# nadeemlab/DeepLIIF

Hardware: AMD Instinct MI355X
Metric: 512x512 tiles/s train-step (5G+5D) (higher is better)
Workload: dtype bf16; 1 GPU; DeepLIIF train step, 5x Resnet-9block G + 5x NLayerD(n=4), GAN+SmoothL1+Adam (BASELINE configs[2] per GPU); tile=512x512x3, batch_per_gpu=8, global_batch=8, norm=instance, precision_policy=bf16, parallelism=dp1, rccl_ranks=1, backend=nccl, streams=3

## Files before the change

deepliif_amd/csrc/conv_s2f.hip:

```cpp
#include "conv_args.h"

__device__ __attribute__((aligned(64))) unsigned char g_s2f_zero_page[64];

constexpr int S2F_MAX_OFF = 9;
struct S2fArgs {
    ConvArgs a;
    int n_off;
    int off_delta[S2F_MAX_OFF];
    int8_t off_dh[S2F_MAX_OFF], off_dw[S2F_MAX_OFF];
    int user_k[S2F_MAX_OFF][4];
};

__device__ __forceinline__ float s2f_row16_sum(float v) {
    v += __builtin_bit_cast(float, __builtin_amdgcn_update_dpp(0, __builtin_bit_cast(int, v), 0xB1, 0xf, 0xf, false));
    v += __builtin_bit_cast(float, __builtin_amdgcn_update_dpp(0, __builtin_bit_cast(int, v), 0x4E, 0xf, 0xf, false));
    v += __builtin_bit_cast(float, __builtin_amdgcn_update_dpp(0, __builtin_bit_cast(int, v), 0x141, 0xf, 0xf, false));
    v += __builtin_bit_cast(float, __builtin_amdgcn_update_dpp(0, __builtin_bit_cast(int, v), 0x140, 0xf, 0xf, false));
    return v;
}

constexpr int S2F_XB = 256 * 128;
constexpr int S2F_WB = 64 * 128;
constexpr int S2F_BUF = S2F_XB + 4 * S2F_WB;
constexpr size_t S2F_LOOP_LDS = (size_t)2 * S2F_BUF;
constexpr size_t S2F_EPI_LDS = (size_t)256 * 512 + 256 * sizeof(int) + (size_t)4 * 2 * 64 * sizeof(float);
constexpr size_t S2F_LDS = S2F_LOOP_LDS > S2F_EPI_LDS ? S2F_LOOP_LDS : S2F_EPI_LDS;

__global__ void __launch_bounds__(512) conv_s2f_kernel(const S2fArgs sa) {
    const ConvArgs &a = sa.a;
    extern __shared__ __attribute__((aligned(16))) char smem_raw[];
    lds_char_t *lds = (lds_char_t *)smem_raw;

    const int tid = threadIdx.x, lane = tid & 63;
    const int wave = __builtin_amdgcn_readfirstlane(tid >> 6);
    const int wm = wave & 3, wn = wave >> 2;
    const int bid = xcd_remap(blockIdx.x, gridDim.x);
    const int tn = bid % a.tiles_n, tm = bid / a.tiles_n;
    const int nch = a.Ci >> 6;
    const int NO = sa.n_off;
    const int T = nch * NO;

    const int lrow = lane >> 3, lcp = lane & 7;
    const int HWq = a.Hq * a.Wq;
    const bf16_t *in = reinterpret_cast<const bf16_t *>(a.in);
    const bf16_t *zero = reinterpret_cast<const bf16_t *>(g_s2f_zero_page);
    const bf16_t *x_ptr[4];
    unsigned x_mask[4];
#pragma unroll
    for (int i = 0; i < 4; ++i) {
        const int s = (wave * 4 + i) * 8 + lrow;
        const int m = tm * 256 + s;
        const bool ok = m < a.Mtot;
        const int mm = ok ? m : 0;
        const int n = mm / HWq, rem = mm - n * HWq;
        const int hq = rem / a.Wq, wq = rem - hq * a.Wq;
        x_ptr[i] = in + ((size_t)(n * a.Hi + hq) * a.Wi + wq) * (size_t)a.in_pstride + (lcp ^ ((s >> 1) & 7)) * 8;
        unsigned mk = 0;
        if (ok)
            for (int o = 0; o < NO; ++o) {
                const int hi = hq + sa.off_dh[o], wi = wq + sa.off_dw[o];
                if (((unsigned)hi < (unsigned)a.Hi) && ((unsigned)wi < (unsigned)a.Wi)) mk |= 1u << o;
            }
        x_mask[i] = mk;
    }
    const int wrow = wave * 8 + lrow;
    const bf16_t *w_ptr = a.w_hi + (size_t)(tn * 64 + wrow) * a.w_kstride + (lcp ^ ((wrow >> 1) & 7)) * 8;

    auto stage = [&](int u) __attribute__((always_inline)) {
        const int c = u / NO, o = u - c * NO;
        const int buf = (u & 1) * S2F_BUF;
        const ptrdiff_t xd = (ptrdiff_t)sa.off_delta[o] + c * 64;
#pragma unroll
        for (int i = 0; i < 4; ++i) {
            const bool ok = (x_mask[i] >> o) & 1u;
            const bf16_t *src = ok ? x_ptr[i] + xd : zero;
            __builtin_amdgcn_global_load_lds((const __attribute__((address_space(1))) void *)src,
                                             (__attribute__((address_space(3))) void *)(lds + buf + (wave * 4 + i) * 1024), 16, 0, 0);
        }
#pragma unroll
        for (int p = 0; p < 4; ++p) {
            const int kb = sa.user_k[o][p];
            if (kb >= 0)
                __builtin_amdgcn_global_load_lds((const __attribute__((address_space(1))) void *)(w_ptr + kb + c * 64),
                                                 (__attribute__((address_space(3))) void *)(lds + buf + S2F_XB + p * S2F_WB + wave * 1024), 16, 0, 0);
        }
    };

    const int lr = lane & 31, lh = lane >> 5;
    const int ax = (wm * 64 + lr) * 128 + ((lh ^ ((lr >> 1) & 7)) << 4);
    const int aw = S2F_XB + (wn * 32 + lr) * 128 + ((lh ^ ((lr >> 1) & 7)) << 4);

    f32x16_t acc[4][2];
#pragma unroll
    for (int p = 0; p < 4; ++p)
#pragma unroll
        for (int j = 0; j < 2; ++j)
#pragma unroll
            for (int r = 0; r < 16; ++r) acc[p][j][r] = 0.f;

    if (T > 0) stage(0);
    for (int u = 0; u < T; ++u) {
        asm volatile("s_waitcnt vmcnt(0)\n\ts_barrier" ::: "memory");
        if (u + 1 < T) stage(u + 1);
        const int c = u / NO, o = u - c * NO;
        (void)c;
        const int buf = (u & 1) * S2F_BUF;
        bf16x8_t xf[4][2];
#pragma unroll
        for (int s = 0; s < 4; ++s)
#pragma unroll
            for (int j = 0; j < 2; ++j) xf[s][j] = *reinterpret_cast<lds_frag_t *>(lds + buf + (ax ^ (s << 5)) + j * 4096);
#pragma unroll
        for (int p = 0; p < 4; ++p) {
            if (sa.user_k[o][p] < 0) continue;
            bf16x8_t wf[4];
#pragma unroll
            for (int s = 0; s < 4; ++s) wf[s] = *reinterpret_cast<lds_frag_t *>(lds + buf + p * S2F_WB + (aw ^ (s << 5)));
#pragma unroll
            for (int s = 0; s < 4; ++s)
#pragma unroll
                for (int j = 0; j < 2; ++j) acc[p][j] = dl_mfma32(wf[s], xf[s][j], acc[p][j]);
        }
    }
    asm volatile("s_waitcnt vmcnt(0) lgkmcnt(0)" ::: "memory");
    __syncthreads();

    lds_char_t *tile = lds;
    __attribute__((address_space(3))) int *rowtab = reinterpret_cast<__attribute__((address_space(3))) int *>(lds + 256 * 512);
    __attribute__((address_space(3))) float *red = reinterpret_cast<__attribute__((address_space(3))) float *>(lds + 256 * 512 + 256 * 4);
    const bool want_stats = a.stats_part != nullptr;
    if (tid < 256) {
        const int m = tm * 256 + tid;
        int opix = -1;
        if (m < a.Mtot) {
            const int n = m / HWq, rem = m - n * HWq;
            const int hq = rem / a.Wq, wq = rem - hq * a.Wq;
            opix = (n * a.Ho + 2 * hq) * a.Wo + 2 * wq;
        }
        rowtab[tid] = opix;
    }
    bool live[2];
#pragma unroll
    for (int j = 0; j < 2; ++j) live[j] = tm * 256 + wm * 64 + j * 32 + lr < a.Mtot;
#pragma unroll
    for (int q = 0; q < 4; ++q) {
        const int cl = wn * 32 + q * 8 + lh * 4;
        const int co = tn * 64 + cl;
        float bias[4] = {0.f, 0.f, 0.f, 0.f};
        if (a.bias) {
#pragma unroll
            for (int e = 0; e < 4; ++e) bias[e] = (co + e < a.bias_n) ? a.bias[co + e] : 0.f;
        }
        float s1[4] = {0.f, 0.f, 0.f, 0.f}, s2[4] = {0.f, 0.f, 0.f, 0.f};
#pragma unroll
        for (int p = 0; p < 4; ++p) {
            const int vch = p * 64 + cl;
            const int unit = (vch >> 2) ^ (((lr & 15) << 1) & 62);
#pragma unroll
            for (int j = 0; j < 2; ++j) {
                float v[4];
#pragma unroll
                for (int e = 0; e < 4; ++e) v[e] = acc[p][j][q * 4 + e] + bias[e];
                if (a.act == DL_ACT_RELU) {
#pragma unroll
                    for (int e = 0; e < 4; ++e) v[e] = v[e] > 0.f ? v[e] : 0.f;
                }
                u32x2_t pk;
                pk[0] = pack2_bf16(v[0], v[1]);
                pk[1] = pack2_bf16(v[2], v[3]);
                *reinterpret_cast<__attribute__((address_space(3))) u32x2_t *>(tile + (wm * 64 + j * 32 + lr) * 512 + unit * 8) = pk;
                if (want_stats && live[j]) {
                    const float q0 = h16_lo_f32(pk[0]), q1 = h16_hi_f32(pk[0]);
                    const float q2 = h16_lo_f32(pk[1]), q3 = h16_hi_f32(pk[1]);
                    s1[0] += q0; s2[0] += q0 * q0; s1[1] += q1; s2[1] += q1 * q1;
                    s1[2] += q2; s2[2] += q2 * q2; s1[3] += q3; s2[3] += q3 * q3;
                }
            }
        }
        if (want_stats) {
#pragma unroll
            for (int e = 0; e < 4; ++e) {
                s1[e] = s2f_row16_sum(s1[e]); s2[e] = s2f_row16_sum(s2[e]);
                s1[e] += __shfl_xor(s1[e], 16, 64); s2[e] += __shfl_xor(s2[e], 16, 64);
            }
            if (lr == 0) {
#pragma unroll
                for (int e = 0; e < 4; ++e) {
                    red[(wm * 2 + 0) * 64 + cl + e] = s1[e];
                    red[(wm * 2 + 1) * 64 + cl + e] = s2[e];
                }
            }
        }
    }
    __syncthreads();
    bf16_t *out = reinterpret_cast<bf16_t *>(a.out);
#pragma unroll 4
    for (int idx = tid; idx < 256 * 32; idx += 512) {
        const int row = idx >> 5, cc = idx & 31;
        const int opix = rowtab[row];
        const int p = cc >> 3, co = tn * 64 + (cc & 7) * 8;
        if (opix < 0 || co >= a.Co) continue;
        const int unit = (cc * 2) ^ (((row & 15) << 1) & 62);
        const u32x4_t v = *reinterpret_cast<__attribute__((address_space(3))) const u32x4_t *>(tile + row * 512 + unit * 8);
        *reinterpret_cast<u32x4_t *>(out + ((size_t)opix + (size_t)(p >> 1) * a.Wo + (p & 1)) * a.out_pstride + co) = v;
    }
    if (want_stats && tid < 64) {
        const int m0 = tm * 256;
        const int n = m0 / HWq;
        const int chunk = (m0 - n * HWq) >> 8;
        const int co = tn * 64 + tid;
        if (co < a.Co) {
            float t1 = 0.f, t2 = 0.f;
#pragma unroll
            for (int w = 0; w < 4; ++w) { t1 += red[(w * 2 + 0) * 64 + tid]; t2 += red[(w * 2 + 1) * 64 + tid]; }
            float *o = a.stats_part + ((size_t)(n * a.stats_nchunks + chunk) * 2) * a.Co + co;
            o[0] = t1;
            o[a.Co] = t2;
        }
    }
}

static bool s2f_phase_order_ok(const ConvArgs &a) {
    for (int p = 0; p < 4; ++p)
        if (a.phase_oh[p] != (p >> 1) || a.phase_ow[p] != (p & 1)) return false;
    return true;
}

bool s2f_eligible(const ConvArgs &a) {
    if (a.n_phase != 4 || a.splitk != 1 || a.raw_out || a.in_step != 1 || a.out_step != 2 || !s2f_phase_order_ok(a)) return false;
    if (a.Ho != 2 * a.Hq || a.Wo != 2 * a.Wq || a.Hi != a.Hq || a.Wi != a.Wq) return false;
    if (a.Ci < 64 || (a.Ci & 63) || a.Co < 64 || (a.Co & 63) || a.pad_mode != DL_PAD_ZERO || a.bn_y != nullptr || a.in_act != DL_ACT_NONE) return false;
    if (a.act != DL_ACT_NONE && a.act != DL_ACT_RELU) return false;
    if (a.epi_old) return false;
    const char *env = dl_switch(DL_SW_CONV_S2F);
    if (a.Mtot < 65536 && !(env && env[0] == '2')) return false;
    int ndist = 0;
    int16_t seen[S2F_MAX_OFF + 1];
    for (int t = 0; t < a.phase_tap_begin[4]; ++t) {
        bool dup = false;
        for (int i = 0; i < ndist; ++i) dup |= seen[i] == a.taps[t];
        if (!dup) {
            if (ndist == S2F_MAX_OFF) return false;
            seen[ndist++] = a.taps[t];
        }
    }
    for (int p = 0; p < 4; ++p)
        for (int t = a.phase_tap_begin[p]; t < a.phase_tap_begin[p + 1]; ++t)
            for (int t2 = t + 1; t2 < a.phase_tap_begin[p + 1]; ++t2)
                if (a.taps[t] == a.taps[t2]) return false;
    return ndist > 0;
}

int s2f_stats_chunks(const ConvArgs &a) {
    const int hw = a.Hq * a.Wq;
    return (hw % 256) ? 0 : hw / 256;
}

int launch_conv_s2f(const ConvArgs &a0, hipStream_t stream) {
    S2fArgs sa;
    memset(&sa, 0, sizeof(sa));
    sa.a = a0;
    ConvArgs &a = sa.a;
    a.tiles_m = (a.Mtot + 255) / 256;
    a.tiles_n = a.Co / 64;
    int no = 0;
    int16_t key[S2F_MAX_OFF];
    for (int p = 0; p < 4; ++p)
        for (int t = a.phase_tap_begin[p]; t < a.phase_tap_begin[p + 1]; ++t) {
            int o = -1;
            for (int i = 0; i < no; ++i)
                if (key[i] == a.taps[t]) o = i;
            if (o < 0) {
                o = no++;
                key[o] = a.taps[t];
                sa.off_dh[o] = tap_dh(a.taps[t]);
                sa.off_dw[o] = tap_dw(a.taps[t]);
                sa.off_delta[o] = ((int)sa.off_dh[o] * a.Wi + (int)sa.off_dw[o]) * a.in_pstride;
                for (int q = 0; q < 4; ++q) sa.user_k[o][q] = -1;
            }
            sa.user_k[o][p] = a.phase_kbase[p] + (t - a.phase_tap_begin[p]) * a.Ci;
        }
    sa.n_off = no;
    if (dl_lds_limit(reinterpret_cast<const void *>(conv_s2f_kernel), S2F_LDS, "dl_conv_forward(s2f)")) return -1;
    dim3 grid(a.tiles_m * a.tiles_n, 1);
    hipLaunchKernelGGL(conv_s2f_kernel, grid, dim3(512), S2F_LDS, stream, sa);
    DL_CHECK_LAUNCH("dl_conv_forward(s2f)");
    return 0;
}
```

Before: 117.5 tiles/s.

## Stage one shared input slab per channel chunk in stride-2 fused conv

```diff
diff --git a/deepliif_amd/csrc/conv_s2f.hip b/deepliif_amd/csrc/conv_s2f.hip
--- a/deepliif_amd/csrc/conv_s2f.hip
+++ b/deepliif_amd/csrc/conv_s2f.hip
@@ -1,14 +1,17 @@
 #include "conv_args.h"
+#include "s2f_plan.h"
 
 __device__ __attribute__((aligned(64))) unsigned char g_s2f_zero_page[64];
 
-constexpr int S2F_MAX_OFF = 9;
 struct S2fArgs {
     ConvArgs a;
     int n_off;
     int off_delta[S2F_MAX_OFF];
-    int8_t off_dh[S2F_MAX_OFF], off_dw[S2F_MAX_OFF];
+    int off_dh[S2F_MAX_OFF], off_dw[S2F_MAX_OFF];
     int user_k[S2F_MAX_OFF][4];
+    int slab, slab_rows, w_base, zero_row;
+    int off_row[S2F_MAX_OFF];
+    int w_lds[S2F_MAX_OFF][4];
 };
 
 __device__ __forceinline__ float s2f_row16_sum(float v) {
@@ -18,13 +21,6 @@
     v += __builtin_bit_cast(float, __builtin_amdgcn_update_dpp(0, __builtin_bit_cast(int, v), 0x140, 0xf, 0xf, false));
     return v;
 }
-
-constexpr int S2F_XB = 256 * 128;
-constexpr int S2F_WB = 64 * 128;
-constexpr int S2F_BUF = S2F_XB + 4 * S2F_WB;
-constexpr size_t S2F_LOOP_LDS = (size_t)2 * S2F_BUF;
-constexpr size_t S2F_EPI_LDS = (size_t)256 * 512 + 256 * sizeof(int) + (size_t)4 * 2 * 64 * sizeof(float);
-constexpr size_t S2F_LDS = S2F_LOOP_LDS > S2F_EPI_LDS ? S2F_LOOP_LDS : S2F_EPI_LDS;
 
 __global__ void __launch_bounds__(512) conv_s2f_kernel(const S2fArgs sa) {
     const ConvArgs &a = sa.a;
@@ -44,51 +40,12 @@
     const int HWq = a.Hq * a.Wq;
     const bf16_t *in = reinterpret_cast<const bf16_t *>(a.in);
     const bf16_t *zero = reinterpret_cast<const bf16_t *>(g_s2f_zero_page);
-    const bf16_t *x_ptr[4];
-    unsigned x_mask[4];
-#pragma unroll
-    for (int i = 0; i < 4; ++i) {
-        const int s = (wave * 4 + i) * 8 + lrow;
-        const int m = tm * 256 + s;
-        const bool ok = m < a.Mtot;
-        const int mm = ok ? m : 0;
-        const int n = mm / HWq, rem = mm - n * HWq;
-        const int hq = rem / a.Wq, wq = rem - hq * a.Wq;
-        x_ptr[i] = in + ((size_t)(n * a.Hi + hq) * a.Wi + wq) * (size_t)a.in_pstride + (lcp ^ ((s >> 1) & 7)) * 8;
-        unsigned mk = 0;
-        if (ok)
-            for (int o = 0; o < NO; ++o) {
-                const int hi = hq + sa.off_dh[o], wi = wq + sa.off_dw[o];
-                if (((unsigned)hi < (unsigned)a.Hi) && ((unsigned)wi < (unsigned)a.Wi)) mk |= 1u << o;
-            }
-        x_mask[i] = mk;
-    }
     const int wrow = wave * 8 + lrow;
     const bf16_t *w_ptr = a.w_hi + (size_t)(tn * 64 + wrow) * a.w_kstride + (lcp ^ ((wrow >> 1) & 7)) * 8;
 
-    auto stage = [&](int u) __attribute__((always_inline)) {
-        const int c = u / NO, o = u - c * NO;
-        const int buf = (u & 1) * S2F_BUF;
-        const ptrdiff_t xd = (ptrdiff_t)sa.off_delta[o] + c * 64;
-#pragma unroll
-        for (int i = 0; i < 4; ++i) {
-            const bool ok = (x_mask[i] >> o) & 1u;
-            const bf16_t *src = ok ? x_ptr[i] + xd : zero;
-            __builtin_amdgcn_global_load_lds((const __attribute__((address_space(1))) void *)src,
-                                             (__attribute__((address_space(3))) void *)(lds + buf + (wave * 4 + i) * 1024), 16, 0, 0);
-        }
-#pragma unroll
-        for (int p = 0; p < 4; ++p) {
-            const int kb = sa.user_k[o][p];
-            if (kb >= 0)
-                __builtin_amdgcn_global_load_lds((const __attribute__((address_space(1))) void *)(w_ptr + kb + c * 64),
-                                                 (__attribute__((address_space(3))) void *)(lds + buf + S2F_XB + p * S2F_WB + wave * 1024), 16, 0, 0);
-        }
-    };
-
     const int lr = lane & 31, lh = lane >> 5;
     const int ax = (wm * 64 + lr) * 128 + ((lh ^ ((lr >> 1) & 7)) << 4);
-    const int aw = S2F_XB + (wn * 32 + lr) * 128 + ((lh ^ ((lr >> 1) & 7)) << 4);
+    const int aw = (wn * 32 + lr) * 128 + ((lh ^ ((lr >> 1) & 7)) << 4);
 
     f32x16_t acc[4][2];
 #pragma unroll
@@ -98,28 +55,157 @@
 #pragma unroll
             for (int r = 0; r < 16; ++r) acc[p][j][r] = 0.f;
 
-    if (T > 0) stage(0);
-    for (int u = 0; u < T; ++u) {
-        asm volatile("s_waitcnt vmcnt(0)\n\ts_barrier" ::: "memory");
-        if (u + 1 < T) stage(u + 1);
-        const int c = u / NO, o = u - c * NO;
-        (void)c;
-        const int buf = (u & 1) * S2F_BUF;
-        bf16x8_t xf[4][2];
-#pragma unroll
-        for (int s = 0; s < 4; ++s)
-#pragma unroll
-            for (int j = 0; j < 2; ++j) xf[s][j] = *reinterpret_cast<lds_frag_t *>(lds + buf + (ax ^ (s << 5)) + j * 4096);
-#pragma unroll
-        for (int p = 0; p < 4; ++p) {
-            if (sa.user_k[o][p] < 0) continue;
-            bf16x8_t wf[4];
-#pragma unroll
-            for (int s = 0; s < 4; ++s) wf[s] = *reinterpret_cast<lds_frag_t *>(lds + buf + p * S2F_WB + (aw ^ (s << 5)));
+    if (!sa.slab) {
+        const bf16_t *x_ptr[4];
+        unsigned x_mask[4];
+#pragma unroll
+        for (int i = 0; i < 4; ++i) {
+            const int s = (wave * 4 + i) * 8 + lrow;
+            const int m = tm * 256 + s;
+            const bool ok = m < a.Mtot;
+            const int mm = ok ? m : 0;
+            const int n = mm / HWq, rem = mm - n * HWq;
+            const int hq = rem / a.Wq, wq = rem - hq * a.Wq;
+            x_ptr[i] = in + ((size_t)(n * a.Hi + hq) * a.Wi + wq) * (size_t)a.in_pstride + (lcp ^ ((s >> 1) & 7)) * 8;
+            unsigned mk = 0;
+            if (ok)
+                for (int o = 0; o < NO; ++o) {
+                    const int hi = hq + sa.off_dh[o], wi = wq + sa.off_dw[o];
+                    mk |= (unsigned)(((unsigned)hi < (unsigned)a.Hi) & ((unsigned)wi < (unsigned)a.Wi)) << o;
+                }
+            x_mask[i] = mk;
+        }
+        auto stage = [&](int u) __attribute__((always_inline)) {
+            const int c = u / NO, o = u - c * NO;
+            const int buf = (u & 1) * S2F_BUF;
+            const ptrdiff_t xd = (ptrdiff_t)sa.off_delta[o] + c * 64;
+#pragma unroll
+            for (int i = 0; i < 4; ++i) {
+                const bool ok = (x_mask[i] >> o) & 1u;
+                const bf16_t *src = ok ? x_ptr[i] + xd : zero;
+                __builtin_amdgcn_global_load_lds((const __attribute__((address_space(1))) void *)src,
+                                                 (__attribute__((address_space(3))) void *)(lds + buf + (wave * 4 + i) * 1024), 16, 0, 0);
+            }
+#pragma unroll
+            for (int p = 0; p < 4; ++p) {
+                const int kb = sa.user_k[o][p];
+                if (kb >= 0)
+                    __builtin_amdgcn_global_load_lds((const __attribute__((address_space(1))) void *)(w_ptr + kb + c * 64),
+                                                     (__attribute__((address_space(3))) void *)(lds + buf + S2F_XB + p * S2F_WB + wave * 1024), 16, 0, 0);
+            }
+        };
+
+        if (T > 0) stage(0);
+        for (int u = 0; u < T; ++u) {
+            asm volatile("s_waitcnt vmcnt(0)\n\ts_barrier" ::: "memory");
+            if (u + 1 < T) stage(u + 1);
+            const int c = u / NO, o = u - c * NO;
+            (void)c;
+            const int buf = (u & 1) * S2F_BUF;
+            bf16x8_t xf[4][2];
 #pragma unroll
             for (int s = 0; s < 4; ++s)
 #pragma unroll
-                for (int j = 0; j < 2; ++j) acc[p][j] = dl_mfma32(wf[s], xf[s][j], acc[p][j]);
+                for (int j = 0; j < 2; ++j) xf[s][j] = *reinterpret_cast<lds_frag_t *>(lds + buf + (ax ^ (s << 5)) + j * 4096);
+#pragma unroll
+            for (int p = 0; p < 4; ++p) {
+                if (sa.user_k[o][p] < 0) continue;
+                bf16x8_t wf[4];
+#pragma unroll
+                for (int s = 0; s < 4; ++s) wf[s] = *reinterpret_cast<lds_frag_t *>(lds + buf + S2F_XB + p * S2F_WB + (aw ^ (s << 5)));
+#pragma unroll
+                for (int s = 0; s < 4; ++s)
+#pragma unroll
+                    for (int j = 0; j < 2; ++j) acc[p][j] = dl_mfma32(wf[s], xf[s][j], acc[p][j]);
+            }
+        }
+    } else {
+        const int slab_b = sa.slab_rows * S2F_ROW_B;
+        const int npieces = sa.slab_rows >> 3;
+        const int ipw = (npieces + 7) >> 3;
+        const int srow = wave * 8 + lrow;
+        const long long f0 = (long long)tm * 256 - sa.off_row[0] + (int)sa.off_dh[0] * a.Wq + (int)sa.off_dw[0] + srow;
+        const long long f_end = (long long)a.N * a.Hi * a.Wi;
+        const int xswz = (lcp ^ ((srow >> 1) & 7)) * 8;
+        auto stage_slab = [&](int c, int i) __attribute__((always_inline)) {
+            const int q = wave + 8 * i;
+            if (q >= npieces) return;
+            const long long f = f0 + 64 * i;
+            const bf16_t *src = (f >= 0 && f < f_end) ? in + f * a.in_pstride + xswz + c * 64 : zero;
+            __builtin_amdgcn_global_load_lds((const __attribute__((address_space(1))) void *)src,
+                                             (__attribute__((address_space(3))) void *)(lds + (c & 1) * slab_b + q * 1024), 16, 0, 0);
+        };
+        auto stage_w = [&](int u) __attribute__((always_inline)) {
+            const int c = u / NO, o = u - c * NO;
+#pragma unroll
+            for (int p = 0; p < 4; ++p) {
+                const int kb = sa.user_k[o][p];
+                if (kb >= 0)
+                    __builtin_amdgcn_global_load_lds((const __attribute__((address_space(1))) void *)(w_ptr + kb + c * 64),
+                                                     (__attribute__((address_space(3))) void *)(lds + sa.w_base + sa.w_lds[o][p] + wave * 1024), 16, 0, 0);
+            }
+        };
+        unsigned f_mask[2];
+#pragma unroll
+        for (int j = 0; j < 2; ++j) {
+            const int m = tm * 256 + wm * 64 + j * 32 + lr;
+            unsigned mk = 0;
+            if (m < a.Mtot) {
+                const int n = m / HWq, rem = m - n * HWq;
+                const int hq = rem / a.Wq, wq = rem - hq * a.Wq;
+                for (int o = 0; o < NO; ++o) {
+                    const int hi = hq + sa.off_dh[o], wi = wq + sa.off_dw[o];
+                    mk |= (unsigned)(((unsigned)hi < (unsigned)a.Hi) & ((unsigned)wi < (unsigned)a.Wi)) << o;
+                }
+            }
+            f_mask[j] = mk;
+        }
+        if (tid < 8) *reinterpret_cast<__attribute__((address_space(3))) u32x4_t *>(lds + sa.zero_row + tid * 16) = u32x4_t{0u, 0u, 0u, 0u};
+        if (T > 0) {
+            for (int i = 0; i < ipw; ++i) stage_slab(0, i);
+            stage_w(0);
+        }
+        __syncthreads();
+        int pend = 0;
+        for (int u = 0; u < T; ++u) {
+            switch (pend) {
+            case 0: asm volatile("s_waitcnt vmcnt(0)\n\ts_barrier" ::: "memory"); break;
+            case 1: asm volatile("s_waitcnt vmcnt(1)\n\ts_barrier" ::: "memory"); break;
+            case 2: asm volatile("s_waitcnt vmcnt(2)\n\ts_barrier" ::: "memory"); break;
+            case 3: asm volatile("s_waitcnt vmcnt(3)\n\ts_barrier" ::: "memory"); break;
+            case 4: asm volatile("s_waitcnt vmcnt(4)\n\ts_barrier" ::: "memory"); break;
+            default: asm volatile("s_waitcnt vmcnt(0)\n\ts_barrier" ::: "memory"); break;
+            }
+            const int c = u / NO, o = u - c * NO;
+            if (u + 1 < T) stage_w(u + 1);
+            pend = 0;
+            if (c + 1 < nch && o + 1 < NO)
+                for (int i = o; i < ipw; i += NO - 1)
+                    if (wave + 8 * i < npieces) {
+                        stage_slab(c + 1, i);
+                        ++pend;
+                    }
+            const int row = wm * 64 + lr + sa.off_row[o];
+            const int xa = (c & 1) * slab_b + row * S2F_ROW_B + ((lh ^ ((row >> 1) & 7)) << 4);
+            const int za = sa.zero_row + (lh << 4);
+            bf16x8_t xf[4][2];
+#pragma unroll
+            for (int j = 0; j < 2; ++j) {
+                const int ja = ((f_mask[j] >> o) & 1u) ? xa + j * 4096 : za;
+#pragma unroll
+                for (int s = 0; s < 4; ++s) xf[s][j] = *reinterpret_cast<lds_frag_t *>(lds + (ja ^ (s << 5)));
+            }
+#pragma unroll
+            for (int p = 0; p < 4; ++p) {
+                if (sa.user_k[o][p] < 0) continue;
+                bf16x8_t wf[4];
+#pragma unroll
+                for (int s = 0; s < 4; ++s) wf[s] = *reinterpret_cast<lds_frag_t *>(lds + sa.w_base + sa.w_lds[o][p] + (aw ^ (s << 5)));
+#pragma unroll
+                for (int s = 0; s < 4; ++s)
+#pragma unroll
+                    for (int j = 0; j < 2; ++j) acc[p][j] = dl_mfma32(wf[s], xf[s][j], acc[p][j]);
+            }
         }
     }
     asm volatile("s_waitcnt vmcnt(0) lgkmcnt(0)" ::: "memory");
@@ -281,9 +367,22 @@
             sa.user_k[o][p] = a.phase_kbase[p] + (t - a.phase_tap_begin[p]) * a.Ci;
         }
     sa.n_off = no;
-    if (dl_lds_limit(reinterpret_cast<const void *>(conv_s2f_kernel), S2F_LDS, "dl_conv_forward(s2f)")) return -1;
+    S2fPlan pl = s2f_plan(no, sa.off_dh, sa.off_dw, sa.user_k, a.Wq);
+#ifdef DL_DEV_SWITCHES
+    static const char *no_slab = DL_DEV_ENV("DL_S2F_SLAB");
+    if (no_slab && no_slab[0] == '0') pl = s2f_plan(0, sa.off_dh, sa.off_dw, sa.user_k, a.Wq);
+#endif
+    sa.slab = pl.slab;
+    sa.slab_rows = pl.rows;
+    sa.w_base = pl.w_base;
+    sa.zero_row = pl.zero_row;
+    for (int o = 0; o < no; ++o) {
+        sa.off_row[o] = pl.off_row[o];
+        for (int p = 0; p < 4; ++p) sa.w_lds[o][p] = pl.w_slot[o][p] < 0 ? 0 : pl.w_slot[o][p] * S2F_WB;
+    }
+    if (dl_lds_limit(reinterpret_cast<const void *>(conv_s2f_kernel), pl.lds_bytes, "dl_conv_forward(s2f)")) return -1;
     dim3 grid(a.tiles_m * a.tiles_n, 1);
-    hipLaunchKernelGGL(conv_s2f_kernel, grid, dim3(512), S2F_LDS, stream, sa);
+    hipLaunchKernelGGL(conv_s2f_kernel, grid, dim3(512), pl.lds_bytes, stream, sa);
     DL_CHECK_LAUNCH("dl_conv_forward(s2f)");
     return 0;
 }
diff --git a/deepliif_amd/csrc/s2f_plan.h b/deepliif_amd/csrc/s2f_plan.h
--- /dev/null
+++ b/deepliif_amd/csrc/s2f_plan.h
@@ -0,0 +1,64 @@
+#pragma once
+#include <stddef.h>
+#include <stdint.h>
+
+constexpr int S2F_MAX_OFF = 9;
+constexpr int S2F_ROW_B = 128;
+constexpr int S2F_XB = 256 * S2F_ROW_B;
+constexpr int S2F_WB = 64 * S2F_ROW_B;
+constexpr int S2F_BUF = S2F_XB + 4 * S2F_WB;
+constexpr size_t S2F_EPI_LDS = (size_t)256 * 512 + 256 * sizeof(int) + (size_t)4 * 2 * 64 * sizeof(float);
+constexpr size_t S2F_PER_OFFSET_LDS = (size_t)2 * S2F_BUF > S2F_EPI_LDS ? (size_t)2 * S2F_BUF : S2F_EPI_LDS;
+constexpr size_t S2F_LDS_CAP = (size_t)160 * 1024;
+
+struct S2fPlan {
+    int slab;
+    int rows;
+    int off_row[S2F_MAX_OFF];
+    int n_wslots;
+    int w_slot[S2F_MAX_OFF][4];
+    int w_base, zero_row;
+    size_t lds_bytes;
+};
+
+static inline S2fPlan s2f_plan(int n_off, const int *dh, const int *dw, const int (*used)[4], int wq, size_t cap = S2F_LDS_CAP) {
+    S2fPlan pl = {};
+    pl.lds_bytes = S2F_PER_OFFSET_LDS;
+    for (int o = 0; o < S2F_MAX_OFF; ++o)
+        for (int p = 0; p < 4; ++p) pl.w_slot[o][p] = -1;
+    if (n_off < 2 || n_off > S2F_MAX_OFF || wq < 1) return pl;
+    long long dmin = 0, dmax = 0;
+    for (int o = 0; o < n_off; ++o) {
+        const long long d = (long long)dh[o] * wq + dw[o];
+        if (o == 0 || d < dmin) dmin = d;
+        if (o == 0 || d > dmax) dmax = d;
+    }
+    const long long rows = (256 + (dmax - dmin) + 7) & ~7LL;
+    int cnt[S2F_MAX_OFF];
+    for (int o = 0; o < n_off; ++o) {
+        cnt[o] = 0;
+        for (int p = 0; p < 4; ++p) cnt[o] += used[o][p] >= 0;
+    }
+    int R = 0;
+    for (int o = 0; o < n_off; ++o) {
+        const int pair = cnt[o] + cnt[(o + 1) % n_off];
+        if (pair > R) R = pair;
+    }
+    const bool odd = n_off & 1;
+    if (odd && cnt[0] + cnt[n_off - 1] + cnt[n_off - 2] > R) R = cnt[0] + cnt[n_off - 1] + cnt[n_off - 2];
+    const long long need = 2 * rows * S2F_ROW_B + (long long)R * S2F_WB + S2F_ROW_B;
+    if (need > (long long)cap) return pl;
+    pl.slab = 1;
+    pl.rows = (int)rows;
+    pl.n_wslots = R;
+    for (int o = 0; o < n_off; ++o) {
+        pl.off_row[o] = (int)((long long)dh[o] * wq + dw[o] - dmin);
+        int s = (odd && o == n_off - 1) ? cnt[0] : (o & 1) ? R - cnt[o] : 0;
+        for (int p = 0; p < 4; ++p)
+            if (used[o][p] >= 0) pl.w_slot[o][p] = s++;
+    }
+    pl.w_base = 2 * pl.rows * S2F_ROW_B;
+    pl.zero_row = pl.w_base + R * S2F_WB;
+    pl.lds_bytes = (size_t)need > S2F_EPI_LDS ? (size_t)need : S2F_EPI_LDS;
+    return pl;
+}
diff --git a/deepliif_amd/csrc/s2f_plan_check.cpp b/deepliif_amd/csrc/s2f_plan_check.cpp
--- /dev/null
+++ b/deepliif_amd/csrc/s2f_plan_check.cpp
@@ -0,0 +1,103 @@
+#include <stdio.h>
+#include <string.h>
+#include <string>
+
+#include "s2f_plan.h"
+
+struct Taps {
+    int n_off;
+    int dh[S2F_MAX_OFF], dw[S2F_MAX_OFF];
+    int used[S2F_MAX_OFF][4];
+};
+
+static Taps make_taps(int k) {
+    Taps t;
+    memset(&t, 0, sizeof(t));
+    for (int o = 0; o < S2F_MAX_OFF; ++o)
+        for (int p = 0; p < 4; ++p) t.used[o][p] = -1;
+    for (int p = 0; p < 4; ++p) {
+        const int oh = p >> 1, ow = p & 1;
+        const int h0 = k == 3 ? 0 : oh - 1, h1 = oh;
+        const int w0 = k == 3 ? 0 : ow - 1, w1 = ow;
+        for (int dh = h0; dh <= h1; ++dh)
+            for (int dw = w0; dw <= w1; ++dw) {
+                int o = -1;
+                for (int i = 0; i < t.n_off; ++i)
+                    if (t.dh[i] == dh && t.dw[i] == dw) o = i;
+                if (o < 0) {
+                    o = t.n_off++;
+                    t.dh[o] = dh;
+                    t.dw[o] = dw;
+                }
+                t.used[o][p] = 64 * (p * 4 + o);
+            }
+    }
+    return t;
+}
+
+static std::string check(const Taps &t, int n, int hq, int wq, int want_slab) {
+    const S2fPlan pl = s2f_plan(t.n_off, t.dh, t.dw, t.used, wq);
+    char buf[256];
+    if (pl.slab != want_slab) {
+        snprintf(buf, sizeof(buf), "slab = %d, expected %d (lds %zu)", pl.slab, want_slab, pl.lds_bytes);
+        return buf;
+    }
+    if (pl.lds_bytes > S2F_LDS_CAP || pl.lds_bytes < S2F_EPI_LDS) return "lds_bytes outside [epilogue, one compute unit]";
+    if (!pl.slab) return pl.lds_bytes == S2F_PER_OFFSET_LDS ? "" : "per-offset staging asks for another size";
+    if (pl.rows % 8 || pl.w_base != 2 * pl.rows * S2F_ROW_B || pl.zero_row != pl.w_base + pl.n_wslots * S2F_WB ||
+        (size_t)pl.zero_row + S2F_ROW_B > pl.lds_bytes)
+        return "layout";
+    for (int o = 0; o < t.n_off; ++o) {
+        const int o2 = (o + 1) % t.n_off;
+        for (int p = 0; p < 4; ++p) {
+            if ((t.used[o][p] >= 0) != (pl.w_slot[o][p] >= 0) || pl.w_slot[o][p] >= pl.n_wslots) return "slot range";
+            for (int q = 0; q < 4; ++q)
+                if (q != p && pl.w_slot[o][p] >= 0 && pl.w_slot[o][p] == pl.w_slot[o][q]) return "two taps of one offset share a slot";
+            for (int q = 0; q < 4; ++q)
+                if (pl.w_slot[o][p] >= 0 && pl.w_slot[o][p] == pl.w_slot[o2][q]) return "consecutive offsets share a slot";
+        }
+    }
+    const long long mtot = (long long)n * hq * wq;
+    const long long tiles = (mtot + 255) / 256;
+    for (long long tm = 0; tm < tiles; ++tm) {
+        const long long first = tm * 256 - pl.off_row[0] + (long long)t.dh[0] * wq + t.dw[0];
+        for (int px = 0; px < 256 && tm * 256 + px < mtot; ++px) {
+            const long long m = tm * 256 + px;
+            const int img = (int)(m / ((long long)hq * wq)), rem = (int)(m % ((long long)hq * wq));
+            const int h = rem / wq, w = rem % wq;
+            for (int o = 0; o < t.n_off; ++o) {
+                const int hi = h + t.dh[o], wi = w + t.dw[o];
+                if (hi < 0 || hi >= hq || wi < 0 || wi >= wq) continue;
+                const int row = px + pl.off_row[o];
+                if (row < 0 || row >= pl.rows) return "slab row outside the slab";
+                const long long f = first + row;
+                if (f != ((long long)img * hq + hi) * wq + wi) return "slab row is another pixel";
+                if (f < 0 || f >= mtot) return "slab row outside the tensor";
+            }
+        }
+    }
+    return "";
+}
+
+int main() {
+    struct Case { const char *name; int k, n, hq, wq, want_slab; };
+    const Case cases[] = {
+        {"k3_n8_128x128", 3, 8, 128, 128, 1}, {"k4_n16_128x128", 4, 16, 128, 128, 0}, {"k4_n16_64x64", 4, 16, 64, 64, 1},
+        {"k3_n1_12x20", 3, 1, 12, 20, 1}, {"k3_n3_16x24", 3, 3, 16, 24, 1}, {"k4_n2_16x16", 4, 2, 16, 16, 1}, {"k3_n2_32x8", 3, 2, 32, 8, 1},
+        {"k4_n2_32x8", 4, 2, 32, 8, 1}, {"k3_n1_32x40", 3, 1, 32, 40, 1}, {"k4_n1_32x40", 4, 1, 32, 40, 1},
+        {"k3_n1_300x1", 3, 1, 300, 1, 1}, {"k4_n3_300x1", 4, 3, 300, 1, 1}, {"k3_n3_1x150", 3, 3, 1, 150, 1}, {"k3_n1_4x130", 3, 1, 4, 130, 1},
+        {"k3_n1_2x183", 3, 1, 2, 183, 1}, {"k3_n1_2x184", 3, 1, 2, 184, 0}, {"k4_n1_4x91", 4, 1, 4, 91, 1}, {"k4_n1_4x92", 4, 1, 4, 92, 0}, {"k3_n1_2x512", 3, 1, 2, 512, 0},
+    };
+    int failed = 0;
+    for (const Case &c : cases) {
+        const std::string what = check(make_taps(c.k), c.n, c.hq, c.wq, c.want_slab);
+        if (what.empty()) printf("ok %s\n", c.name);
+        else { printf("FAILED %s: %s\n", c.name, what.c_str()); ++failed; }
+    }
+    Taps one = make_taps(3);
+    one.n_off = 1;
+    const S2fPlan pl = s2f_plan(one.n_off, one.dh, one.dw, one.used, 64);
+    if (pl.slab == 0 && pl.lds_bytes == S2F_PER_OFFSET_LDS) printf("ok one_offset\n");
+    else { printf("FAILED one_offset\n"); ++failed; }
+    return failed;
+}
```

After: 117.5 tiles/s (median of 3 runs). No clear change (+0.0%).
